# Sanoojan/VFace

Measured on AMD Instinct MI355X. Metric: swapped frames/sec at 512x512, 50-step DDIM, higher is better.
Workload: dtype f16

## Files before the change

vface_amd/csrc/stfront.hip:

```cpp
#include "common.hpp"
#include "launch.hpp"
#include "vface_kernels.hpp"

namespace {

constexpr int sf_ring(int n, int want) { for (int r = want; r > 1; --r) if (n % r == 0) return r; return 1; }

template <class TT, int C>
__global__ __launch_bounds__(256, 1) void st_front_kernel(StFrontParams p) {
    using E = typename TT::elem;
    using V8 = typename TT::v8;
    using V4 = typename TT::v4;
    constexpr int KS = C / 16;
    constexpr int TIN = C / 32;
    constexpr int NW = 4;
    constexpr int WE = 32 * C;
    constexpr int OPS = C / 64;
    constexpr int RA = sf_ring(KS, 5);
    constexpr int SPF = 36;
    constexpr int SPH = 40;
    static_assert(C % 64 == 0 && C <= 320, "C: a multiple of 64, at most 320");
    constexpr int LASTP = 4 * (OPS - 1) + 1;
    constexpr int PA = 2 < KS ? 2 : KS - 1, PB = 6 < KS ? 6 : KS - 1;
    constexpr bool ST_AFTER = PB >= LASTP;
    extern __shared__ __attribute__((aligned(16))) unsigned char smem_raw[];
    E* sW = reinterpret_cast<E*>(smem_raw);
    float* sBin = reinterpret_cast<float*>(sW + NW * WE);
    float* sGam = sBin + C;
    float* sBet = sGam + C;
    float* sA = sBet + C;
    float* sB = sA + C;
    float* scrAll = sB + C;

    const int t_ = threadIdx.x, lane = t_ & 63;
    const int wave = __builtin_amdgcn_readfirstlane(t_ >> 6);
    const int fr = lane & 31, fh = lane >> 5;
    float* scr = scrAll + wave * (32 * SPF);
    E* scrh = reinterpret_cast<E*>(scr);

    const int tilesA = p.rows_full / 128, tilesT = p.M / 128;
    const bool inA = (int)blockIdx.x < p.gridA;
    const int t_first = inA ? (int)blockIdx.x : tilesA + ((int)blockIdx.x - p.gridA);
    const int t_stride = inA ? p.gridA : ((int)gridDim.x - p.gridA);
    const int t_end = inA ? tilesA : tilesT;
    const int qf = inA ? 0 : p.nq_lo / 32;
    const int TQ = p.NQ / 32 - qf;
    const int S = TIN + TQ;
    if (t_first >= t_end) return;

    for (int i = t_; i < C / 4; i += 256) {
        reinterpret_cast<float4*>(sBin)[i] = reinterpret_cast<const float4*>(p.b_in)[i];
        reinterpret_cast<float4*>(sGam)[i] = reinterpret_cast<const float4*>(p.gamma)[i];
        reinterpret_cast<float4*>(sBet)[i] = reinterpret_cast<const float4*>(p.beta)[i];
    }

    const i32x4_t rW = raw_buffer_rsrc(p.Wcat, (unsigned)((C + p.NQ) * C) * 2u);
    const unsigned ldsW = lds_addr_of(sW);
    constexpr int SPR = C / 8;
    int w_off[OPS];
#pragma unroll
    for (int i = 0; i < OPS; ++i) {
        const int id = (wave * OPS + i) * 64 + lane;
        const int r1 = id / SPR, s1 = id - r1 * SPR;
        const int c1 = (s1 & ~7) | ((s1 & 7) ^ ((r1 >> 1) & 7));
        w_off[i] = (r1 * C + c1 * 8) * 2;
    }
    const unsigned ldsWw = ldsW + (unsigned)(wave * OPS * 1024);
    int wi_s = 0, wi_glob = 0, wi_slot = 0;
    auto issue_piece = [&](int i) { raw_lds_dma16(rW, ldsWw + (unsigned)(wi_slot * (WE * 2) + i * 1024), w_off[i], wi_glob); };
    auto advance_issue = [&]() {
        ++wi_s;
        wi_glob += 32 * C * 2;
        if (wi_s == TIN) wi_glob += qf * (32 * C * 2);
        if (wi_s == S) { wi_s = 0; wi_glob = 0; }
        wi_slot = (wi_slot + 1) & (NW - 1);
    };
    int w_lane[4];
#pragma unroll
    for (int j = 0; j < 4; ++j) w_lane[j] = fr * C + (((2 * j + fh) ^ ((fr >> 1) & 7)) << 3);
    auto frag_at = [&](const E* const (&base)[4], int ks) -> V8 { return *reinterpret_cast<const V8*>(base[ks & 3] + (ks >> 2) * 64); };
    int wr_slot = 1;
    const E* wa[4];
    const E* wb[4];
#pragma unroll
    for (int j = 0; j < 4; ++j) { wa[j] = sW + w_lane[j]; wb[j] = sW + WE + w_lane[j]; }

    __syncthreads();
#pragma unroll
    for (int g = 0; g < 3; ++g) {
#pragma unroll
        for (int i = 0; i < OPS; ++i) issue_piece(i);
        advance_issue();
    }
    asm volatile("s_waitcnt vmcnt(0)" ::: "memory");
    raw_barrier();
    V8 af[RA];
#pragma unroll
    for (int i = 0; i < RA; ++i) af[i] = frag_at(wa, i);

    f16_t out[TIN];

    auto stage_tail = [&]() {
        advance_issue();
        wr_slot = (wr_slot + 1) & (NW - 1);
#pragma unroll
        for (int j = 0; j < 4; ++j) { wa[j] = wb[j]; wb[j] = sW + wr_slot * WE + w_lane[j]; }
    };
#define SF_STAGE_TOP(NWAIT)                                                   \
    asm volatile("s_waitcnt vmcnt(%0)" ::"n"(NWAIT) : "memory");             \
    raw_barrier();
#define SF_KLOOP(MFMA_CALL)                                                                                              \
    _Pragma("unroll") for (int ks = 0; ks < KS; ++ks) {                                                                  \
        MFMA_CALL;                                                                                                       \
        af[(ks + RA - 1) % RA] = (ks - 1 + RA < KS) ? frag_at(wa, ks - 1 + RA) : frag_at(wb, ks - 1 + RA - KS);          \
        if (ks % 4 == 1) issue_piece(ks / 4);                                                                            \
        __builtin_amdgcn_sched_barrier(0);                                                                               \
    }

    V8 xf[KS];
    for (int tile = t_first; tile < t_end; tile += t_stride) {
        const long tok0 = (long)tile * 128 + wave * 32;
        {
            const int img = (int)(((long)tile * 128) / p.hw);
            const float* abp = p.ab + (long)img * p.ld_ab * 2;
            __syncthreads();
            for (int c = t_; c < C; c += 256) {
                const float2 v = *reinterpret_cast<const float2*>(abp + 2 * c);
                sA[c] = v.x; sB[c] = v.y;
            }
            float v[KS][8];
            const float* xr = p.x32 + (tok0 + fr) * p.ldx + fh * 8;
#pragma unroll
            for (int ks = 0; ks < KS; ++ks) {
                const float4 a = *reinterpret_cast<const float4*>(xr + ks * 16);
                const float4 b = *reinterpret_cast<const float4*>(xr + ks * 16 + 4);
                v[ks][0] = a.x; v[ks][1] = a.y; v[ks][2] = a.z; v[ks][3] = a.w; v[ks][4] = b.x; v[ks][5] = b.y; v[ks][6] = b.z; v[ks][7] = b.w;
            }
            __syncthreads();
#pragma unroll
            for (int ks = 0; ks < KS; ++ks) {
                const float* ap = sA + ks * 16 + fh * 8;
                const float* bp = sB + ks * 16 + fh * 8;
                const float4 a0 = *reinterpret_cast<const float4*>(ap), a1 = *reinterpret_cast<const float4*>(ap + 4);
                const float4 b0 = *reinterpret_cast<const float4*>(bp), b1 = *reinterpret_cast<const float4*>(bp + 4);
                const float am[8] = {a0.x, a0.y, a0.z, a0.w, a1.x, a1.y, a1.z, a1.w};
                const float bm[8] = {b0.x, b0.y, b0.z, b0.w, b1.x, b1.y, b1.z, b1.w};
                V8 o;
#pragma unroll
                for (int j = 0; j < 8; ++j) o[j] = from_f32<E>(v[ks][j] * am[j] + bm[j]);
                xf[ks] = o;
            }
#pragma unroll
            for (int ks = 0; ks < KS; ++ks) asm volatile("" : "+v"(xf[ks]));
            gap_valu_result_to_mfma(xf[KS - 1]);
        }
        auto t0_to_scratch = [&](int ot) {
#pragma unroll
            for (int q4 = 0; q4 < 4; ++q4)
                *reinterpret_cast<float4*>(scr + fr * SPF + q4 * 8 + fh * 4) =
                    make_float4(out[ot][4 * q4], out[ot][4 * q4 + 1], out[ot][4 * q4 + 2], out[ot][4 * q4 + 3]);
        };
        auto t0_scratch_to_global = [&](int ot) {
#pragma unroll
            for (int k = 0; k < 4; ++k) {
                const int it = lane + 64 * k, tok = it >> 3, ch = it & 7;
                const float4 vv = *reinterpret_cast<const float4*>(scr + tok * SPF + ch * 4);
                *reinterpret_cast<float4*>(p.t0 + (tok0 + tok) * p.ldt0 + ot * 32 + ch * 4) = vv;
            }
        };
#pragma unroll
        for (int ot = 0; ot < TIN; ++ot) {
            if (ot == 0) { SF_STAGE_TOP(OPS) }
            else if (ot == 1) { SF_STAGE_TOP(OPS) }
            else if (ot == 2) { SF_STAGE_TOP(OPS + 4) }
            else { SF_STAGE_TOP(OPS + 4 + (ST_AFTER ? 4 : 0)) }
            {
                const float* bp = sBin + ot * 32 + fh * 4;
#pragma unroll
                for (int q4 = 0; q4 < 4; ++q4) {
                    const float4 b = *reinterpret_cast<const float4*>(bp + q4 * 8);
                    out[ot][4 * q4] = b.x; out[ot][4 * q4 + 1] = b.y; out[ot][4 * q4 + 2] = b.z; out[ot][4 * q4 + 3] = b.w;
                }
                gap_valu_result_to_acc_mfma(out[ot]);
            }
#pragma unroll
            for (int ks = 0; ks < KS; ++ks) {
                TT::mfma32x32_acc(out[ot], af[ks % RA], xf[ks]);
                af[(ks + RA - 1) % RA] = (ks - 1 + RA < KS) ? frag_at(wa, ks - 1 + RA) : frag_at(wb, ks - 1 + RA - KS);
                if (ks % 4 == 1) issue_piece(ks / 4);
                if (ot > 0 && ks == PA) t0_to_scratch(ot - 1);
                if (ot > 0 && ks == PB) t0_scratch_to_global(ot - 1);
                __builtin_amdgcn_sched_barrier(0);
            }
            stage_tail();
        }
        {
#pragma unroll
            for (int ot = 0; ot < TIN; ++ot) gap_acc_result_to_valu(out[ot]);
            float s = 0.f;
#pragma unroll
            for (int ot = 0; ot < TIN; ++ot)
#pragma unroll
                for (int q = 0; q < 16; ++q) s += out[ot][q];
            s += __shfl_xor(s, 32, 64);
            const float mean = s / (float)C;
            float qq = 0.f;
#pragma unroll
            for (int ot = 0; ot < TIN; ++ot)
#pragma unroll
                for (int q = 0; q < 16; ++q) { const float d = out[ot][q] - mean; qq += d * d; }
            qq += __shfl_xor(qq, 32, 64);
            const float rstd = rsqrtf(qq / (float)C + p.eps);
            t0_to_scratch(TIN - 1);
            t0_scratch_to_global(TIN - 1);
            asm volatile("" ::: "memory");
#pragma unroll
            for (int ot = 0; ot < TIN; ++ot) {
                const float* gp = sGam + ot * 32 + fh * 4;
                const float* bp = sBet + ot * 32 + fh * 4;
#pragma unroll
                for (int j = 0; j < 2; ++j) {
                    V8 o;
#pragma unroll
                    for (int e4 = 0; e4 < 2; ++e4) {
                        const int q4 = 2 * j + e4;
                        const float4 g = *reinterpret_cast<const float4*>(gp + q4 * 8), b = *reinterpret_cast<const float4*>(bp + q4 * 8);
                        o[4 * e4 + 0] = from_f32<E>((out[ot][4 * q4 + 0] - mean) * rstd * g.x + b.x);
                        o[4 * e4 + 1] = from_f32<E>((out[ot][4 * q4 + 1] - mean) * rstd * g.y + b.y);
                        o[4 * e4 + 2] = from_f32<E>((out[ot][4 * q4 + 2] - mean) * rstd * g.z + b.z);
                        o[4 * e4 + 3] = from_f32<E>((out[ot][4 * q4 + 3] - mean) * rstd * g.w + b.w);
                    }
                    xf[2 * ot + j] = o;
                }
                if (p.ln) {
                    E* lnp = reinterpret_cast<E*>(p.ln);
#pragma unroll
                    for (int q4 = 0; q4 < 4; ++q4) {
                        V4 h4;
#pragma unroll
                        for (int e = 0; e < 4; ++e) h4[e] = xf[2 * ot + (q4 >> 1)][4 * (q4 & 1) + e];
                        *reinterpret_cast<V4*>(scrh + fr * SPH + q4 * 8 + fh * 4) = h4;
                    }
#pragma unroll
                    for (int k = 0; k < 2; ++k) {
                        const int it = lane + 64 * k, tok = it >> 2, ch = it & 3;
                        const V8 vv = *reinterpret_cast<const V8*>(scrh + tok * SPH + ch * 8);
                        *reinterpret_cast<V8*>(lnp + (tok0 + tok) * p.ldln + ot * 32 + ch * 8) = vv;
                    }
                }
            }
#pragma unroll
            for (int ks = 0; ks < KS; ++ks) asm volatile("" : "+v"(xf[ks]));
            gap_valu_result_to_mfma(xf[KS - 1]);
        }
        asm volatile("" ::: "memory");
        E* qp = reinterpret_cast<E*>(p.qkv);
        V4 hprev[4];
        auto q_to_scratch = [&]() {
#pragma unroll
            for (int q4 = 0; q4 < 4; ++q4) *reinterpret_cast<V4*>(scrh + fr * SPH + q4 * 8 + fh * 4) = hprev[q4];
        };
        auto q_scratch_to_global = [&](int qt_) {
            const int col0 = (qf + qt_) * 32;
#pragma unroll
            for (int k = 0; k < 2; ++k) {
                const int it = lane + 64 * k, tok = it >> 2, ch = it & 3;
                const V8 vv = *reinterpret_cast<const V8*>(scrh + tok * SPH + ch * 8);
                *reinterpret_cast<V8*>(qp + (tok0 + tok) * p.ldq + col0 + ch * 8) = vv;
            }
        };
        for (int qt = 0; qt < TQ; ++qt) {
            if (qt == 0) { SF_STAGE_TOP(0) } else if (qt == 1) { SF_STAGE_TOP(OPS) } else if (qt == 2) { SF_STAGE_TOP(OPS + 2) }
            else { SF_STAGE_TOP(OPS + 2 + (ST_AFTER ? 2 : 0)) }
            f16_t acc;
            TT::mfma32x32_vzero(acc, af[0], xf[0]);
            af[(RA - 1) % RA] = (RA - 1 < KS) ? frag_at(wa, RA - 1) : frag_at(wb, RA - 1 - KS);
            __builtin_amdgcn_sched_barrier(0);
#pragma unroll
            for (int ks = 1; ks < KS; ++ks) {
                TT::mfma32x32_vacc(acc, af[ks % RA], xf[ks]);
                af[(ks + RA - 1) % RA] = (ks - 1 + RA < KS) ? frag_at(wa, ks - 1 + RA) : frag_at(wb, ks - 1 + RA - KS);
                if (ks % 4 == 1) issue_piece(ks / 4);
                if (qt > 0 && ks == PA) q_to_scratch();
                if (qt > 0 && ks == PB) q_scratch_to_global(qt - 1);
                __builtin_amdgcn_sched_barrier(0);
            }
            stage_tail();
            gap_mfma_result_to_valu(acc);
#pragma unroll
            for (int q4 = 0; q4 < 4; ++q4)
#pragma unroll
                for (int e = 0; e < 4; ++e) hprev[q4][e] = from_f32<E>(acc[4 * q4 + e]);
        }
        q_to_scratch();
        q_scratch_to_global(TQ - 1);
        asm volatile("" ::: "memory");
    }
    asm volatile("s_waitcnt vmcnt(0)" ::: "memory");
#undef SF_STAGE_TOP
#undef SF_KLOOP
}

template <class TT, int C>
int launch_c(const StFrontParams& p0, hipStream_t stream) {
    StFrontParams p = p0;
    constexpr size_t lds = (size_t)4 * 32 * C * 2 + (size_t)5 * C * 4 + (size_t)4 * 32 * 36 * 4;
    auto kern = st_front_kernel<TT, C>;
    static VfOncePerDevice attr_set;
    if (lds > 64 * 1024 && !attr_set.set_lds(reinterpret_cast<const void*>(kern), (int)lds)) return VF_ERR_LAUNCH;
    int dev = 0, ncu = 256;
    if (hipGetDevice(&dev) == hipSuccess) {
        int v = 0;
        if (hipDeviceGetAttribute(&v, hipDeviceAttributeMultiprocessorCount, dev) == hipSuccess && v > 0) ncu = v;
    }
    const int tilesA = p.rows_full / 128, tilesB = p.M / 128 - tilesA;
    const long workA = (long)tilesA * (C / 32 + p.NQ / 32), workB = (long)tilesB * (C / 32 + (p.NQ - p.nq_lo) / 32);
    int grid = (int)((tilesA + tilesB) < ncu ? (tilesA + tilesB) : ncu);
    int gridA = 0;
    if (tilesA > 0 && tilesB > 0) {
        gridA = (int)((grid * workA + (workA + workB) / 2) / (workA + workB));
        if (gridA < 1) gridA = 1;
        if (gridA > tilesA) gridA = tilesA;
        if (grid - gridA > tilesB) grid = gridA + tilesB;
        if (grid - gridA < 1) gridA = grid - 1;
    } else if (tilesA > 0) {
        gridA = grid;
    }
    p.gridA = gridA;
    hipLaunchKernelGGL(kern, dim3(grid), dim3(256), lds, stream, p);
    return vf_launched();
}

template <class TT>
int launch_t(const StFrontParams& p, hipStream_t stream) {
    switch (p.C) {
        case 64: return launch_c<TT, 64>(p, stream);
        case 128: return launch_c<TT, 128>(p, stream);
        case 320: return launch_c<TT, 320>(p, stream);
        default: return VF_ERR_SHAPE;
    }
}

}

bool vf_st_front_supported(long M, int C, int hw) {
    return M > 0 && (M % 128) == 0 && hw > 0 && (hw % 128) == 0 && (M % hw) == 0 && (C == 64 || C == 128 || C == 320);
}

int vf_launch_st_front(const StFrontParams& p, int dtype, hipStream_t stream) {
    if (!p.x32 || !p.ab || !p.Wcat || !p.b_in || !p.gamma || !p.beta || !p.t0 || !p.qkv) return VF_ERR_ARG;
    if (!vf_st_front_supported(p.M, p.C, p.hw)) return VF_ERR_SHAPE;
    if (p.NQ <= 0 || (p.NQ % 32) || p.nq_lo < 0 || (p.nq_lo % 32) || p.nq_lo >= p.NQ || p.rows_full < 0 || p.rows_full > p.M ||
        (p.rows_full % 128) || (p.rows_full == 0 && p.nq_lo == 0)) return VF_ERR_SHAPE;
    if ((p.ldx & 3) || (p.ldt0 & 3) || (p.ldq & 7) || (p.ln && (p.ldln & 7)) || p.ld_ab < p.C) return VF_ERR_ALIGN;
    if (((uintptr_t)p.x32 | (uintptr_t)p.ab | (uintptr_t)p.Wcat | (uintptr_t)p.b_in | (uintptr_t)p.gamma | (uintptr_t)p.beta |
         (uintptr_t)p.t0 | (uintptr_t)p.qkv | (uintptr_t)p.ln) & 15) return VF_ERR_ALIGN;
    if (dtype == VF_DTYPE_F16) return launch_t<F16>(p, stream);
    if (dtype == VF_DTYPE_BF16) return launch_t<BF16>(p, stream);
    return VF_ERR_DTYPE;
}
```

Before: 8.302.

## Prefetch next tile's activations via LDS DMA during Q-projection MFMA stages

Replaces the per-tile synchronous global load of x (and the affine scale/shift vectors) with async buffer-to-LDS DMA of 64-channel chunks. The chunks for the next tile are issued and converted inside the current tile's MFMA stages, and the results are kept in a second register set. The next image's scale/shift values are also loaded early and written to shared memory after the LN phase, which removes two barriers from the tile start. The aim is to hide the x load latency behind compute, at the cost of extra LDS, more registers and more complex wait-count scheduling.

```diff
diff --git a/vface_amd/csrc/stfront.hip b/vface_amd/csrc/stfront.hip
--- a/vface_amd/csrc/stfront.hip
+++ b/vface_amd/csrc/stfront.hip
@@ -23,6 +23,13 @@
     constexpr int LASTP = 4 * (OPS - 1) + 1;
     constexpr int PA = 2 < KS ? 2 : KS - 1, PB = 6 < KS ? 6 : KS - 1;
     constexpr bool ST_AFTER = PB >= LASTP;
+    constexpr int NCH = C / 64, XOPS = 8;
+    constexpr int XR0 = KS >= 16 ? 4 : 0, XRS = KS >= 16 ? 3 : (KS >= 8 ? 2 : 1), XCV = KS >= 8 ? 1 : 0;
+    constexpr int XP = KS >= 16 ? 2 : 3, XD = KS >= 16 ? 0 : 1, XIK = KS >= 16 ? 15 : 0;
+    constexpr int QU = NCH > 1 ? XP * (NCH - 2) + XD + 3 : 1;
+    static_assert(NCH == 1 || XIK < LASTP, "an x chunk is issued before the last weight piece of its stage");
+    static_assert(XR0 + 3 * XRS + XCV < KS, "a chunk is read inside one stage");
+    static_assert(NCH == 1 || XD > 0 || XIK > XR0 + 3 * XRS + XCV, "the chunk buffer is free when the next chunk is issued");
     extern __shared__ __attribute__((aligned(16))) unsigned char smem_raw[];
     E* sW = reinterpret_cast<E*>(smem_raw);
     float* sBin = reinterpret_cast<float*>(sW + NW * WE);
@@ -31,6 +38,7 @@
     float* sA = sBet + C;
     float* sB = sA + C;
     float* scrAll = sB + C;
+    float* sXAll = scrAll + 4 * (32 * SPF);
 
     const int t_ = threadIdx.x, lane = t_ & 63;
     const int wave = __builtin_amdgcn_readfirstlane(t_ >> 6);
@@ -53,6 +61,51 @@
         reinterpret_cast<float4*>(sGam)[i] = reinterpret_cast<const float4*>(p.gamma)[i];
         reinterpret_cast<float4*>(sBet)[i] = reinterpret_cast<const float4*>(p.beta)[i];
     }
+    {
+        const float* abp = p.ab + (((long)t_first * 128) / p.hw) * p.ld_ab * 2;
+        for (int c = t_; c < C; c += 256) {
+            const float2 v = *reinterpret_cast<const float2*>(abp + 2 * c);
+            sA[c] = v.x; sB[c] = v.y;
+        }
+    }
+
+    const unsigned ldsX = lds_addr_of(sXAll) + (unsigned)(wave * (32 * 64 * 4));
+    const float* sX = sXAll + wave * (32 * 64);
+    const int x_ld4 = p.ldx * 4;
+    auto x_rsrc = [&](long tok) { return raw_buffer_rsrc(p.x32 + tok * p.ldx, (unsigned)(31 * p.ldx + C) * 4u); };
+    auto x_issue = [&](const i32x4_t& rX, int c) {
+        int l = lane;
+        asm volatile("" : "+v"(l));
+#pragma unroll
+        for (int i = 0; i < XOPS; ++i) {
+            const int r = 4 * i + (l >> 4);
+            raw_lds_dma16(rX, ldsX + (unsigned)(i * 1024), r * x_ld4 + (((l & 15) ^ (r & 15)) << 4), c * 256);
+        }
+    };
+    struct XT { float4 v0, v1, a0, a1, b0, b1; };
+    const int x_q0 = fr * 64 + ((((2 * fh) ^ (fr & 15))) << 2);
+    auto x_read = [&](int c, int j, XT& t) {
+        int q = x_q0, h = fh * 8;
+        asm volatile("" : "+v"(q), "+v"(h));
+        const int o = q ^ (16 * j);
+        t.v0 = *reinterpret_cast<const float4*>(sX + o);
+        t.v1 = *reinterpret_cast<const float4*>(sX + (o ^ 4));
+        const float* ap = sA + (h + c * 64 + j * 16);
+        const float* bp = sB + (h + c * 64 + j * 16);
+        t.a0 = *reinterpret_cast<const float4*>(ap); t.a1 = *reinterpret_cast<const float4*>(ap + 4);
+        t.b0 = *reinterpret_cast<const float4*>(bp); t.b1 = *reinterpret_cast<const float4*>(bp + 4);
+    };
+    auto x_conv = [&](const XT& t) -> V8 {
+        const float v[8] = {t.v0.x, t.v0.y, t.v0.z, t.v0.w, t.v1.x, t.v1.y, t.v1.z, t.v1.w};
+        const float am[8] = {t.a0.x, t.a0.y, t.a0.z, t.a0.w, t.a1.x, t.a1.y, t.a1.z, t.a1.w};
+        const float bm[8] = {t.b0.x, t.b0.y, t.b0.z, t.b0.w, t.b1.x, t.b1.y, t.b1.z, t.b1.w};
+        V8 o;
+#pragma unroll
+        for (int j = 0; j < 8; ++j) o[j] = from_f32<E>(v[j] * am[j] + bm[j]);
+        return o;
+    };
+    auto xcs = [](int c) { return c == 0 ? 0 : XP * (c - 1) + XD + 2; };
+    auto xis = [](int c) { return XP * (c - 1) + XD; };
 
     const i32x4_t rW = raw_buffer_rsrc(p.Wcat, (unsigned)((C + p.NQ) * C) * 2u);
     const unsigned ldsW = lds_addr_of(sW);
@@ -118,37 +171,33 @@
     }
 
     V8 xf[KS];
+    V8 nxf[KS];
+#pragma unroll
+    for (int ks = 0; ks < KS; ++ks) nxf[ks] = V8{};
+    int nxq = 0;
     for (int tile = t_first; tile < t_end; tile += t_stride) {
         const long tok0 = (long)tile * 128 + wave * 32;
+        const bool pf = tile + t_stride < t_end;
+        const long tok0n = tok0 + (long)t_stride * 128;
+        const i32x4_t rXn = x_rsrc(pf ? tok0n : tok0);
         {
-            const int img = (int)(((long)tile * 128) / p.hw);
-            const float* abp = p.ab + (long)img * p.ld_ab * 2;
-            __syncthreads();
-            for (int c = t_; c < C; c += 256) {
-                const float2 v = *reinterpret_cast<const float2*>(abp + 2 * c);
-                sA[c] = v.x; sB[c] = v.y;
-            }
-            float v[KS][8];
-            const float* xr = p.x32 + (tok0 + fr) * p.ldx + fh * 8;
-#pragma unroll
-            for (int ks = 0; ks < KS; ++ks) {
-                const float4 a = *reinterpret_cast<const float4*>(xr + ks * 16);
-                const float4 b = *reinterpret_cast<const float4*>(xr + ks * 16 + 4);
-                v[ks][0] = a.x; v[ks][1] = a.y; v[ks][2] = a.z; v[ks][3] = a.w; v[ks][4] = b.x; v[ks][5] = b.y; v[ks][6] = b.z; v[ks][7] = b.w;
-            }
-            __syncthreads();
-#pragma unroll
-            for (int ks = 0; ks < KS; ++ks) {
-                const float* ap = sA + ks * 16 + fh * 8;
-                const float* bp = sB + ks * 16 + fh * 8;
-                const float4 a0 = *reinterpret_cast<const float4*>(ap), a1 = *reinterpret_cast<const float4*>(ap + 4);
-                const float4 b0 = *reinterpret_cast<const float4*>(bp), b1 = *reinterpret_cast<const float4*>(bp + 4);
-                const float am[8] = {a0.x, a0.y, a0.z, a0.w, a1.x, a1.y, a1.z, a1.w};
-                const float bm[8] = {b0.x, b0.y, b0.z, b0.w, b1.x, b1.y, b1.z, b1.w};
-                V8 o;
-#pragma unroll
-                for (int j = 0; j < 8; ++j) o[j] = from_f32<E>(v[ks][j] * am[j] + bm[j]);
-                xf[ks] = o;
+            const i32x4_t rX = x_rsrc(tok0);
+#pragma unroll
+            for (int c = 0; c < NCH; ++c) {
+                if (c < nxq) {
+#pragma unroll
+                    for (int j = 0; j < 4; ++j) xf[4 * c + j] = nxf[4 * c + j];
+                } else {
+                    asm volatile("s_waitcnt lgkmcnt(0)" ::: "memory");
+                    x_issue(rX, c);
+                    asm volatile("s_waitcnt vmcnt(0)" ::: "memory");
+#pragma unroll
+                    for (int j = 0; j < 4; ++j) {
+                        XT t;
+                        x_read(c, j, t);
+                        xf[4 * c + j] = x_conv(t);
+                    }
+                }
             }
 #pragma unroll
             for (int ks = 0; ks < KS; ++ks) asm volatile("" : "+v"(xf[ks]));
@@ -187,6 +236,7 @@
             for (int ks = 0; ks < KS; ++ks) {
                 TT::mfma32x32_acc(out[ot], af[ks % RA], xf[ks]);
                 af[(ks + RA - 1) % RA] = (ks - 1 + RA < KS) ? frag_at(wa, ks - 1 + RA) : frag_at(wb, ks - 1 + RA - KS);
+                if (ot == TIN - 1 && ks == 0) { if (pf) x_issue(rXn, 0); }
                 if (ks % 4 == 1) issue_piece(ks / 4);
                 if (ot > 0 && ks == PA) t0_to_scratch(ot - 1);
                 if (ot > 0 && ks == PB) t0_scratch_to_global(ot - 1);
@@ -197,6 +247,13 @@
         {
 #pragma unroll
             for (int ot = 0; ot < TIN; ++ot) gap_acc_result_to_valu(out[ot]);
+            float2 abn[(C + 255) / 256] = {};
+            if (pf) {
+                const float* abp = p.ab + (((long)(tile + t_stride) * 128) / p.hw) * p.ld_ab * 2;
+#pragma unroll
+                for (int i = 0; i < (C + 255) / 256; ++i)
+                    if (t_ + 256 * i < C) abn[i] = *reinterpret_cast<const float2*>(abp + 2 * (t_ + 256 * i));
+            }
             float s = 0.f;
 #pragma unroll
             for (int ot = 0; ot < TIN; ++ot)
@@ -252,6 +309,12 @@
 #pragma unroll
             for (int ks = 0; ks < KS; ++ks) asm volatile("" : "+v"(xf[ks]));
             gap_valu_result_to_mfma(xf[KS - 1]);
+            if (pf) {
+#pragma unroll
+                for (int i = 0; i < (C + 255) / 256; ++i)
+                    if (t_ + 256 * i < C) { sA[t_ + 256 * i] = abn[i].x; sB[t_ + 256 * i] = abn[i].y; }
+                __syncthreads();
+            }
         }
         asm volatile("" ::: "memory");
         E* qp = reinterpret_cast<E*>(p.qkv);
@@ -269,20 +332,33 @@
                 *reinterpret_cast<V8*>(qp + (tok0 + tok) * p.ldq + col0 + ch * 8) = vv;
             }
         };
-        for (int qt = 0; qt < TQ; ++qt) {
-            if (qt == 0) { SF_STAGE_TOP(0) } else if (qt == 1) { SF_STAGE_TOP(OPS) } else if (qt == 2) { SF_STAGE_TOP(OPS + 2) }
+        auto q_stage = [&](const int qt, const int xc, const int xi, const int xp) __attribute__((always_inline)) {
+            const bool xw = xp >= 0 && pf && xcs(xp) < TQ;
+            if (qt == 0) { SF_STAGE_TOP(0) }
+            else if (qt == 1) { if (xw) { SF_STAGE_TOP(OPS + XOPS) } else { SF_STAGE_TOP(OPS) } }
+            else if (qt == 2) { if (xw) { SF_STAGE_TOP(OPS + 2 + XOPS) } else { SF_STAGE_TOP(OPS + 2) } }
+            else if (xw) { SF_STAGE_TOP(OPS + 2 + (ST_AFTER ? 2 : 0) + XOPS) }
             else { SF_STAGE_TOP(OPS + 2 + (ST_AFTER ? 2 : 0)) }
+            const bool xon = xc >= 0 && pf, xgo = xi >= 0 && pf && xcs(xi) < TQ;
+            XT xt;
             f16_t acc;
-            TT::mfma32x32_vzero(acc, af[0], xf[0]);
-            af[(RA - 1) % RA] = (RA - 1 < KS) ? frag_at(wa, RA - 1) : frag_at(wb, RA - 1 - KS);
-            __builtin_amdgcn_sched_barrier(0);
-#pragma unroll
-            for (int ks = 1; ks < KS; ++ks) {
-                TT::mfma32x32_vacc(acc, af[ks % RA], xf[ks]);
+#pragma unroll
+            for (int ks = 0; ks < KS; ++ks) {
+                if (ks == 0) TT::mfma32x32_vzero(acc, af[0], xf[0]);
+                else TT::mfma32x32_vacc(acc, af[ks % RA], xf[ks]);
                 af[(ks + RA - 1) % RA] = (ks - 1 + RA < KS) ? frag_at(wa, ks - 1 + RA) : frag_at(wb, ks - 1 + RA - KS);
                 if (ks % 4 == 1) issue_piece(ks / 4);
                 if (qt > 0 && ks == PA) q_to_scratch();
                 if (qt > 0 && ks == PB) q_scratch_to_global(qt - 1);
+                if (xc >= 0) {
+#pragma unroll
+                    for (int j = 0; j < 4; ++j) {
+                        if (XCV > 0 && ks == XR0 + XRS * j + XCV) { if (xon) { nxf[4 * (xc < 0 ? 0 : xc) + j] = x_conv(xt); asm volatile("" : "+a"(nxf[4 * (xc < 0 ? 0 : xc) + j])); } }
+                        if (ks == XR0 + XRS * j) { if (xon) x_read(xc, j, xt); }
+                        if (XCV == 0 && ks == XR0 + XRS * j) { if (xon) { nxf[4 * (xc < 0 ? 0 : xc) + j] = x_conv(xt); asm volatile("" : "+a"(nxf[4 * (xc < 0 ? 0 : xc) + j])); } }
+                    }
+                }
+                if (xi >= 0 && ks == XIK) { if (xgo) x_issue(rXn, xi); }
                 __builtin_amdgcn_sched_barrier(0);
             }
             stage_tail();
@@ -291,7 +367,22 @@
             for (int q4 = 0; q4 < 4; ++q4)
 #pragma unroll
                 for (int e = 0; e < 4; ++e) hprev[q4][e] = from_f32<E>(acc[4 * q4 + e]);
-        }
+        };
+#pragma unroll
+        for (int qt = 0; qt < QU; ++qt) {
+            int xc = -1, xi = -1, xp = -1;
+#pragma unroll
+            for (int c = 0; c < NCH; ++c) {
+                if (xcs(c) == qt) xc = c;
+                if (c > 0 && xis(c) == qt) xi = c;
+                if (c > 0 && xis(c) == qt - 1) xp = c;
+            }
+            if (qt < TQ) q_stage(qt, xc, xi, xp);
+        }
+        for (int qt = QU; qt < TQ; ++qt) q_stage(qt, -1, -1, -1);
+        nxq = 0;
+#pragma unroll
+        for (int c = 0; c < NCH; ++c) nxq += (pf && xcs(c) < TQ) ? 1 : 0;
         q_to_scratch();
         q_scratch_to_global(TQ - 1);
         asm volatile("" ::: "memory");
@@ -304,7 +395,8 @@
 template <class TT, int C>
 int launch_c(const StFrontParams& p0, hipStream_t stream) {
     StFrontParams p = p0;
-    constexpr size_t lds = (size_t)4 * 32 * C * 2 + (size_t)5 * C * 4 + (size_t)4 * 32 * 36 * 4;
+    constexpr size_t lds = (size_t)4 * 32 * C * 2 + (size_t)5 * C * 4 + (size_t)4 * 32 * 36 * 4 + (size_t)4 * 32 * 64 * 4;
+    static_assert(lds <= 160 * 1024, "LDS of a CU");
     auto kern = st_front_kernel<TT, C>;
     static VfOncePerDevice attr_set;
     if (lds > 64 * 1024 && !attr_set.set_lds(reinterpret_cast<const void*>(kern), (int)lds)) return VF_ERR_LAUNCH;
```

After: 8.305 (median of 2 runs). About the same (+0.0%).
